# kkaytekin/Supervised-Depth-Estimation-from-Polarized-Images

Hardware: AMD Instinct MI355X
Metric: train images/sec (512x612, 3-encoder) (higher is better)
Workload: dtype f32; 1 GPU; BASELINE configs[2]: full 3-encoder (augment_xolp+augment_normals), multi-scale loss scales=[0,1,2,3], batch 16 per GPU, 512x612 frames (network/loss on 512x640 padded), dropout 0.1, Adam lr 1e-4, fp32; global_batch=16, height=512, width=640, frame_width=612, parallelism=dp1

## Files before the change

### supervised-depth-estimation-from-polarized-images_amd/csrc/elementwise.hip

```cpp
#include "pd_common.h"
#include <cstdlib>
#include <cstdint>

namespace {

constexpr int EW_T = 256;

__device__ __forceinline__ float4 ld4(const float* p) { return *reinterpret_cast<const float4*>(p); }
__device__ __forceinline__ void st4(float* p, float4 v) { *reinterpret_cast<float4*>(p) = v; }
typedef float ew_f4 __attribute__((ext_vector_type(4)));
__device__ __forceinline__ void st4_nt(float* p, float4 v) {
    const ew_f4 w = {v.x, v.y, v.z, v.w};
    __builtin_nontemporal_store(w, reinterpret_cast<ew_f4*>(p));
}
__device__ __forceinline__ float4 f4(float v) { return make_float4(v, v, v, v); }

__device__ __forceinline__ uint4 philox4x32_10(uint4 c, uint2 k) {
    const uint32_t M0 = 0xD2511F53u, M1 = 0xCD9E8D57u, W0 = 0x9E3779B9u, W1 = 0xBB67AE85u;
#pragma unroll
    for (int r = 0; r < 10; ++r) {
        const uint32_t hi0 = __umulhi(M0, c.x), lo0 = M0 * c.x;
        const uint32_t hi1 = __umulhi(M1, c.z), lo1 = M1 * c.z;
        c = make_uint4(hi1 ^ c.y ^ k.x, lo1, hi0 ^ c.w ^ k.y, lo0);
        k.x += W0; k.y += W1;
// ... 251 lines not shown
    if (a.pool) {
        const float* p = a.x + (((size_t)n * a.H + 2 * ho) * a.W + 2 * wo) * a.C + c4;
        float4 v[4];
        v[0] = affine4(ld4(p), s, b); v[1] = affine4(ld4(p + a.C), s, b);
        v[2] = affine4(ld4(p + (long)a.W * a.C), s, b); v[3] = affine4(ld4(p + (long)a.W * a.C + a.C), s, b);
        if (a.relu_pre) { v[0] = relu4(v[0]); v[1] = relu4(v[1]); v[2] = relu4(v[2]); v[3] = relu4(v[3]); }
        const int me = ((h & 1) << 1) | (w & 1);
        int ax = 0, ay = 0, az = 0, aw = 0;
        float mx = v[0].x, my = v[0].y, mz = v[0].z, mw = v[0].w;
#pragma unroll
        for (int j = 1; j < 4; ++j) {
            if (v[j].x > mx) { mx = v[j].x; ax = j; }
            if (v[j].y > my) { my = v[j].y; ay = j; }
            if (v[j].z > mz) { mz = v[j].z; az = j; }
            if (v[j].w > mw) { mw = v[j].w; aw = j; }
        }
        g = make_float4(ax == me ? g.x : 0.f, ay == me ? g.y : 0.f, az == me ? g.z : 0.f, aw == me ? g.w : 0.f);
    }
    if (a.relu_pre)
        g = make_float4(z.x > 0.f ? g.x : 0.f, z.y > 0.f ? g.y : 0.f, z.z > 0.f ? g.z : 0.f, z.w > 0.f ? g.w : 0.f);
    return g;
}

template <bool APPLY>
__global__ __launch_bounds__(EW_T) void chain_bwd_kernel(const ChainArgs a) {
    const unsigned cq = a.C >> 2;
    const unsigned total = (unsigned)a.N * a.H * a.W * cq;
    float4 sg = f4(0.f), sgx = f4(0.f);
    const unsigned i0 = blockIdx.x * (unsigned)EW_T + threadIdx.x;
    const int c4 = (int)(i0 % cq) * 4;
    const float4 s = a.scale ? ld4(a.scale + c4) : f4(1.f);
    const float4 b = a.scale ? ld4(a.shift + c4) : f4(0.f);
    const float4 m = a.mean ? ld4(a.mean + c4) : f4(0.f), is = a.mean ? ld4(a.invstd + c4) : f4(0.f);
    const float4 c1 = (APPLY && a.mean) ? ld4(a.coef + c4) : f4(0.f), c2 = (APPLY && a.mean) ? ld4(a.coef + a.C + c4) : f4(0.f);
    if (a.pool && !(a.H & 1) && !(a.W & 1)) {
        const unsigned Ho = a.H >> 1, Wo = a.W >> 1;
        const unsigned wtotal = (unsigned)a.N * Ho * Wo * cq;
        for (unsigned i = i0; i < wtotal; i += gridDim.x * (unsigned)EW_T) {
            const unsigned opix = i / cq;
            const unsigned t = opix / Wo;
            const unsigned wo = opix - t * Wo;
            const unsigned n = t / Ho;
            const unsigned ho = t - n * Ho;
            const size_t p00 = (((size_t)n * a.H + 2 * ho) * a.W + 2 * wo) * a.C + c4;
            const size_t offs[4] = {p00, p00 + a.C, p00 + (size_t)a.W * a.C, p00 + (size_t)a.W * a.C + a.C};
            float4 xv[4], v[4];
#pragma unroll
            for (int j = 0; j < 4; ++j) {
                xv[j] = ld4(a.x + offs[j]);
                v[j] = affine4(xv[j], s, b);
                if (a.relu_pre) v[j] = relu4(v[j]);
            }
            float4 g = ld4(a.dy + (size_t)opix * a.ld_dy + c4);
            if (a.relu_post) {
                const float4 o = ld4(a.out + (size_t)opix * a.ld_out + c4);
                g = make_float4(o.x > 0.f ? g.x : 0.f, o.y > 0.f ? g.y : 0.f, o.z > 0.f ? g.z : 0.f, o.w > 0.f ? g.w : 0.f);
            }
            if (a.drop_p > 0.f) g = mul4(g, dropout_scale(i, a.seed, site_offset(a.offset, a.step_state), a.drop_p));
            int ax = 0, ay = 0, az = 0, aw = 0;
            float mx = v[0].x, my = v[0].y, mz = v[0].z, mw = v[0].w;
#pragma unroll
            for (int j = 1; j < 4; ++j) {
                if (v[j].x > mx) { mx = v[j].x; ax = j; }
                if (v[j].y > my) { my = v[j].y; ay = j; }
                if (v[j].z > mz) { mz = v[j].z; az = j; }
                if (v[j].w > mw) { mw = v[j].w; aw = j; }
            }
            if (a.relu_pre)
                g = make_float4(mx > 0.f ? g.x : 0.f, my > 0.f ? g.y : 0.f, mz > 0.f ? g.z : 0.f, mw > 0.f ? g.w : 0.f);
#pragma unroll
            for (int j = 0; j < 4; ++j) {
                const float4 gj = make_float4(ax == j ? g.x : 0.f, ay == j ? g.y : 0.f, az == j ? g.z : 0.f, aw == j ? g.w : 0.f);
                float4 xh = f4(0.f);
                if (a.mean) xh = make_float4((xv[j].x - m.x) * is.x, (xv[j].y - m.y) * is.y, (xv[j].z - m.z) * is.z, (xv[j].w - m.w) * is.w);
                if (!APPLY) {
                    sg = add4(sg, gj);
                    sgx = add4(sgx, mul4(gj, xh));
                } else {
                    float4 d;
                    if (a.mean) d = make_float4(s.x * (gj.x - c1.x - xh.x * c2.x), s.y * (gj.y - c1.y - xh.y * c2.y),
                                                s.z * (gj.z - c1.z - xh.z * c2.z), s.w * (gj.w - c1.w - xh.w * c2.w));
                    else d = mul4(gj, s);
                    st4_nt(a.dx + offs[j], d);
                }
            }
        }
    } else
    for (unsigned i = i0; i < total; i += gridDim.x * (unsigned)EW_T) {
        const unsigned pix = i / cq;
        const unsigned t = pix / a.W;
        const unsigned w = pix - t * a.W;
        const unsigned n = t / a.H;
        const unsigned h = t - n * a.H;
        const float4 xv = ld4(a.x + (size_t)pix * a.C + c4);
        float4 gp;
        const float4 g = chain_grad(a, n, h, w, c4, xv, s, b, &gp);
        if (APPLY && a.dres) st4(a.dres + (size_t)pix * a.C + c4, gp);
        float4 xh = f4(0.f);
        if (a.mean) xh = make_float4((xv.x - m.x) * is.x, (xv.y - m.y) * is.y, (xv.z - m.z) * is.z, (xv.w - m.w) * is.w);
        if (!APPLY) {
            sg = add4(sg, g);
            sgx = add4(sgx, mul4(g, xh));
        } else {
            float4 d;
            if (a.mean) {
                d = make_float4(s.x * (g.x - c1.x - xh.x * c2.x), s.y * (g.y - c1.y - xh.y * c2.y),
                                s.z * (g.z - c1.z - xh.z * c2.z), s.w * (g.w - c1.w - xh.w * c2.w));
            } else {
                d = mul4(g, s);
            }
            st4_nt(a.dx + (size_t)pix * a.C + c4, d);
        }
    }
    if (!APPLY) {
        __shared__ float red[EW_T][8];
        float* r = red[threadIdx.x];
        r[0] = sg.x; r[1] = sg.y; r[2] = sg.z; r[3] = sg.w; r[4] = sgx.x; r[5] = sgx.y; r[6] = sgx.z; r[7] = sgx.w;
        __syncthreads();
        if ((int)threadIdx.x < cq) {
            float acc8[8] = {0, 0, 0, 0, 0, 0, 0, 0};
            for (int t = threadIdx.x; t < EW_T; t += cq)
#pragma unroll
                for (int j = 0; j < 8; ++j) acc8[j] += red[t][j];
            float* o = a.partial + ((long)blockIdx.x * a.C + 4 * threadIdx.x) * 2;
#pragma unroll
            for (int j = 0; j < 4; ++j) { o[2 * j] = acc8[j]; o[2 * j + 1] = acc8[4 + j]; }
        }
    }
}

__device__ __forceinline__ long divmod(long i, int d, int& rem) {
    if (i >> 32) { const long q = i / d; rem = (int)(i - q * d); return q; }
    const unsigned u = (unsigned)i, q = u / (unsigned)d;
    rem = (int)(u - q * (unsigned)d);
// ... 747 lines not shown
```

### supervised-depth-estimation-from-polarized-images_amd/csrc/loss.hip

```cpp
#include "pd_common.h"
#include <algorithm>
#include <cstdlib>

namespace {

constexpr int LT = 256;

__device__ __forceinline__ float wave_sum(float v) {
#pragma unroll
    for (int o = 32; o > 0; o >>= 1) v += __shfl_xor(v, o);
    return v;
}

template <int K>
__device__ __forceinline__ void block_sum(float (&v)[K], float* smem ) {
#pragma unroll
    for (int k = 0; k < K; ++k) v[k] = wave_sum(v[k]);
    const int lane = threadIdx.x & 63, wave = threadIdx.x >> 6;
    if (lane == 0)
#pragma unroll
        for (int k = 0; k < K; ++k) smem[wave * K + k] = v[k];
    __syncthreads();
    if (threadIdx.x == 0)
#pragma unroll
// ... 600 lines not shown
                                                      int N, long P, int accumulate, unsigned bid, unsigned nb) {
    const long total = N * P;
    for (long i = bid * (long)LT + threadIdx.x; i < total; i += (long)nb * LT) {
        const long n = i / P;
        if (!mean) { gdisp[i] = accumulate ? gdisp[i] + G[i] : G[i]; continue; }
        const float me = mean[n] + 1e-7f;
        const float v = G[i] / me - (float)(gd_acc[n] / ((double)me * me * (double)P));
        gdisp[i] = accumulate ? gdisp[i] + v : v;
    }
}
__global__ __launch_bounds__(LT) void smooth_bwd_final_kernel(const float* __restrict__ G, const float* __restrict__ mean,
                                                              const double* __restrict__ gd_acc, float* __restrict__ gdisp,
                                                              int N, long P, int accumulate) {
    smooth_bwd_final_body(G, mean, gd_acc, gdisp, N, P, accumulate, blockIdx.x, gridDim.x);
}

struct MsArgs {
    int S, N, H, W;
    const float* disp[8]; const float* color[8];
    float* depth[8]; float* mean[8]; float2* edge[8];
    float* gdisp[8]; float* gws[8]; float* gup[8];
    int hs[8], ws[8];
    unsigned nb_full, nb_s[8];
};

__global__ __launch_bounds__(LT) void ms_disp_to_depth_kernel(const MsArgs a, float min_disp, float max_disp) {
    const int s = blockIdx.y;
    disp_to_depth_body(a.disp[s], a.depth[s], nullptr, a.N, a.hs[s], a.ws[s], a.H, a.W, min_disp, max_disp, blockIdx.x, gridDim.x);
}

__global__ __launch_bounds__(LT) void ms_sup_fwd_kernel(const MsArgs a, const float* __restrict__ gt, const float* __restrict__ K,
                                                        const float4* __restrict__ gtn, float* __restrict__ partial,
                                                        int part_stride, float min_d, float max_d, int with_normals) {
    __shared__ float sm[4 * 3];
    const int N = a.N, H = a.H, W = a.W;
    const long total = (long)N * H * W;
    float acc[8][3];
#pragma unroll
    for (int s = 0; s < 8; ++s) { acc[s][0] = 0.f; acc[s][1] = 0.f; acc[s][2] = 0.f; }
    for (long i = blockIdx.x * (long)LT + threadIdx.x; i < total; i += (long)gridDim.x * LT) {
        int x, y;
        const long t = divmod(i, W, x);
        const long n = divmod(t, H, y);
        const float g = gt[i];
        if (!(g >= min_d && g <= max_d)) continue;
        V3 ng{0, 0, 0};
        float n1 = 1.f;
        Cam c{};
        if (with_normals) {
            c = load_cam(K, n);
            if (gtn) { const float4 q = gtn[i]; ng = V3{q.x, q.y, q.z}; }
            else { V3 A, B; float nv; sobel_xyz(gt + n * H * W, H, W, x, y, c, A, B); ng = normalize12(cross(A, B), nv); }
            n1 = fmaxf(sqrtf(dot(ng, ng)), 1e-8f);
        }
#pragma unroll
        for (int s = 0; s < 8; ++s) {
            if (s >= a.S) break;
            const float* pred = a.depth[s];
            acc[s][0] += fabsf(g - pred[i]);
            acc[s][2] += 1.f;
            if (with_normals) {
                V3 A, B; float nv;
                sobel_xyz(pred + n * H * W, H, W, x, y, c, A, B);
                const V3 np_ = normalize12(cross(A, B), nv);
                const float n2 = fmaxf(sqrtf(dot(np_, np_)), 1e-8f);
                const float cs = (ng.x / n1) * (np_.x / n2) + (ng.y / n1) * (np_.y / n2) + (ng.z / n1) * (np_.z / n2);
                acc[s][1] += 2.f - cs;
            }
        }
    }
    for (int s = 0; s < a.S; ++s) {
        float v[3] = {acc[s][0], acc[s][1], acc[s][2]};
        __syncthreads();
        block_sum<3>(v, sm);
        if (threadIdx.x == 0) {
            float* p = partial + ((long)s * part_stride + blockIdx.x) * 3;
            p[0] = v[0]; p[1] = v[1]; p[2] = v[2];
        }
    }
}

__global__ __launch_bounds__(1024) void ms_image_mean_kernel(const MsArgs a) {
    __shared__ double sm[16];
    const int s = blockIdx.y;
    image_mean_body(sm, a.disp[s], a.mean[s], a.hs[s] * a.ws[s], blockIdx.x);
}

__global__ __launch_bounds__(LT) void ms_smooth_fwd_kernel(const MsArgs a, float* __restrict__ partial, int part_stride) {
    __shared__ float sm[4 * 2];
    const int s = blockIdx.y;
    if (blockIdx.x >= a.nb_s[s]) return;
    smooth_fwd_body(sm, a.disp[s], a.color[s], a.mean[s], partial + (long)s * part_stride * 2, a.edge[s], a.N, a.hs[s], a.ws[s],
                    blockIdx.x, a.nb_s[s]);
}

__global__ __launch_bounds__(LT) void ms_sup_bwd_kernel(const MsArgs a, const float* __restrict__ gt, const float* __restrict__ K,
                                                        const float4* __restrict__ gtn, const float* __restrict__ wts,
                                                        const double* __restrict__ sums, float min_d, float max_d,
                                                        float disp_range, int tiles_h, int tiles_w, int ntiles) {
    __shared__ float abl[6][SB_HP];
    const int s = blockIdx.y;
    sup_bwd_fused_body(abl, a.depth[s], gt, K, gtn, wts + 3 * s, sums + 5 * s, a.gup[s], a.N, a.H, a.W, min_d, max_d, disp_range, 1,
                       tiles_h, tiles_w, ntiles, blockIdx.x, gridDim.x);
}

__global__ __launch_bounds__(LT) void ms_up_gather_bwd_kernel(const MsArgs a) {
    const int s = blockIdx.y;
    if (blockIdx.x >= a.nb_s[s]) return;
    const int f = a.H / a.hs[s];
    if (f == 1) up_gather_bwd_f_body<1>(a.gup[s], a.gdisp[s], a.N, a.hs[s], a.ws[s], a.H, a.W, 0, blockIdx.x, a.nb_s[s]);
    else if (f == 2) up_gather_bwd_f_body<2>(a.gup[s], a.gdisp[s], a.N, a.hs[s], a.ws[s], a.H, a.W, 0, blockIdx.x, a.nb_s[s]);
    else if (f == 4) up_gather_bwd_f_body<4>(a.gup[s], a.gdisp[s], a.N, a.hs[s], a.ws[s], a.H, a.W, 0, blockIdx.x, a.nb_s[s]);
    else up_gather_bwd_f_body<8>(a.gup[s], a.gdisp[s], a.N, a.hs[s], a.ws[s], a.H, a.W, 0, blockIdx.x, a.nb_s[s]);
}

__global__ __launch_bounds__(LT) void ms_smooth_bwd_g_kernel(const MsArgs a, const float* __restrict__ wts,
                                                             double* __restrict__ gd_acc) {
    __shared__ double smd[4];
    const int s = blockIdx.y;
    if (blockIdx.x >= a.nb_s[s]) return;
    smooth_bwd_g_body(smd, a.disp[s], a.color[s], a.mean[s], wts + 3 * s, a.edge[s], a.gws[s], gd_acc + (long)s * a.N, a.N,
                      a.hs[s], a.ws[s], blockIdx.x, a.nb_s[s]);
}

__global__ __launch_bounds__(LT) void ms_smooth_bwd_final_kernel(const MsArgs a, const double* __restrict__ gd_acc) {
    const int s = blockIdx.y;
    if (blockIdx.x >= a.nb_s[s]) return;
    smooth_bwd_final_body(a.gws[s], a.mean[s], gd_acc + (long)s * a.N, a.gdisp[s], a.N, (long)a.hs[s] * a.ws[s], 1, blockIdx.x,
                          a.nb_s[s]);
}

struct LossMeta {
    int S;
    int sup_rows[8], sm_rows[8], N[8], h[8], w[8], scale_id[8];
};

__global__ __launch_bounds__(256) void loss_finalize_kernel(const float* __restrict__ sup_part,
                                                            const float* __restrict__ sm_part, const LossMeta m,
                                                            int part_stride, float w_normals, float w_smooth,
                                                            double* __restrict__ sums, float* __restrict__ vals) {
    __shared__ double red[256];
    __shared__ double tot[8 * 5];
    for (int s = 0; s < m.S; ++s) {
        for (int j = 0; j < 5; ++j) {
            double v = 0.0;
            if (j < 3) {
                const float* sp = sup_part + (long)s * part_stride * 3;
                for (int r = threadIdx.x; r < m.sup_rows[s]; r += 256) v += sp[r * 3 + j];
            } else {
                const float* mp = sm_part + (long)s * part_stride * 2;
                for (int r = threadIdx.x; r < m.sm_rows[s]; r += 256) v += mp[r * 2 + (j - 3)];
            }
// ... 52 lines not shown
    wts[3 * s + 2] = gl * w_smooth / (float)(1 << m.scale_id[s]);
}

}

extern "C" int pd_loss_rows(long n) { return (int)lgrid(n); }

extern "C" int pd_disp_to_depth(const void* disp, void* depth, void* updisp, int N, int hs, int ws, int H, int W,
                                float min_depth, float max_depth, void* stream) {
    PD_REQUIRE(disp && depth && N >= 0 && hs > 0 && ws > 0 && H >= hs && W >= ws, "pd_disp_to_depth: bad arguments");
    PD_REQUIRE(min_depth > 0 && max_depth > min_depth, "pd_disp_to_depth: bad depth range");
    if (N == 0) return PD_OK;
    hipLaunchKernelGGL(disp_to_depth_kernel, dim3(lgrid((long)N * H * W)), dim3(LT), 0, (hipStream_t)stream,
                       (const float*)disp, (float*)depth, (float*)updisp, N, hs, ws, H, W, 1.f / max_depth,
                       1.f / min_depth);
    return pd::check_launch("pd_disp_to_depth");
}

extern "C" int pd_up_gather_bwd(const void* gup, void* gdisp, int N, int hs, int ws, int H, int W, int accumulate,
                                int generic, void* stream) {
    PD_REQUIRE(gup && gdisp && N >= 0 && hs > 0 && ws > 0, "pd_up_gather_bwd: bad arguments");
    PD_REQUIRE(H % hs == 0 && W % ws == 0, "pd_up_gather_bwd: full size must be an integer multiple of the scale size");
    if (N == 0) return PD_OK;
    const int f = generic ? 0 : H / hs;
    const unsigned grid = lgrid((long)N * hs * ws);
#define PD_UPG(F) hipLaunchKernelGGL(up_gather_bwd_f_kernel<F>, dim3(grid), dim3(LT), 0, (hipStream_t)stream, \
                                     (const float*)gup, (float*)gdisp, N, hs, ws, H, W, accumulate)
    if (W / ws == f && f == 1) PD_UPG(1);
    else if (W / ws == f && f == 2) PD_UPG(2);
    else if (W / ws == f && f == 4) PD_UPG(4);
    else if (W / ws == f && f == 8) PD_UPG(8);
    else
        hipLaunchKernelGGL(up_gather_bwd_kernel, dim3(grid), dim3(LT), 0, (hipStream_t)stream, (const float*)gup,
                           (float*)gdisp, N, hs, ws, H, W, accumulate);
#undef PD_UPG
    return pd::check_launch("pd_up_gather_bwd");
}

extern "C" int pd_gt_normals(const void* gt, const void* K, void* gtn, int N, int H, int W, float min_depth,
                             float max_depth, void* stream) {
    PD_REQUIRE(gt && K && gtn && N > 0 && H > 0 && W > 0 && pd::aligned16(gtn), "pd_gt_normals: bad arguments");
    hipLaunchKernelGGL(gt_normals_kernel, dim3(lgrid((long)N * H * W)), dim3(LT), 0, (hipStream_t)stream, (const float*)gt,
                       (const float*)K, (float4*)gtn, N, H, W, min_depth, max_depth);
    return pd::check_launch("pd_gt_normals");
}

extern "C" int pd_sup_loss_fwd(const void* pred, const void* gt, const void* K, const void* gt_normals, void* partial, int N,
                               int H, int W, float min_depth, float max_depth, int with_normals, void* stream) {
// ... 90 lines not shown
    const unsigned grid = lgrid((long)N * h * w);
    hipLaunchKernelGGL(smooth_bwd_g_kernel, dim3(grid), dim3(LT), 0, st, (const float*)disp, (const float*)img,
                       (const float*)mean, (const float*)wts, (const float2*)edge_w, (float*)g_ws, (double*)gd_acc, N, h, w);
    hipLaunchKernelGGL(smooth_bwd_final_kernel, dim3(grid), dim3(LT), 0, st, (const float*)g_ws, (const float*)mean,
                       (const double*)gd_acc, (float*)gdisp, N, (long)h * w, accumulate);
    return pd::check_launch("pd_smooth_bwd");
}

static int ms_fill(MsArgs& a, const void* const* disps, const void* const* colors, void* const* depths, void* const* means,
                   void* const* edge_ws, const int* hs, const int* ws, int S, int N, int H, int W) {
    PD_REQUIRE(S > 0 && S <= 8 && N > 0 && H > 0 && W > 0 && disps && depths && hs && ws, "pd_multiscale_loss: bad arguments");
    a = MsArgs{};
    a.S = S; a.N = N; a.H = H; a.W = W;
    a.nb_full = lgrid((long)N * H * W);
    for (int s = 0; s < S; ++s) {
        PD_REQUIRE(disps[s] && depths[s] && hs[s] > 1 && ws[s] > 1 && H % hs[s] == 0 && W % ws[s] == 0 && H / hs[s] == W / ws[s] &&
                       (H / hs[s] == 1 || H / hs[s] == 2 || H / hs[s] == 4 || H / hs[s] == 8),
                   "pd_multiscale_loss: scale %d: the full size must be 1, 2, 4 or 8 times the scale size", s);
        a.disp[s] = (const float*)disps[s]; a.color[s] = colors ? (const float*)colors[s] : nullptr;
        a.depth[s] = (float*)depths[s]; a.mean[s] = means ? (float*)means[s] : nullptr;
        a.edge[s] = edge_ws ? (float2*)edge_ws[s] : nullptr;
        a.hs[s] = hs[s]; a.ws[s] = ws[s];
        a.nb_s[s] = lgrid((long)N * hs[s] * ws[s]);
    }
    return PD_OK;
}

extern "C" int pd_multiscale_loss_fwd(const void* const* disps, const void* const* colors, const int* hs, const int* ws, int S,
                                      const void* gt, const void* K, const void* gt_normals, void* const* depths,
                                      void* const* means, void* const* edge_ws, void* sup_part, void* sm_part, int part_stride,
                                      int N, int H, int W, float min_depth, float max_depth, int with_normals, void* stream) {
    MsArgs a;
    int rc = ms_fill(a, disps, colors, depths, means, edge_ws, hs, ws, S, N, H, W);
    if (rc) return rc;
    PD_REQUIRE(colors && means && gt && (K || !with_normals) && sup_part && sm_part, "pd_multiscale_loss_fwd: null pointer");
    PD_REQUIRE(min_depth > 0 && max_depth > min_depth, "pd_multiscale_loss_fwd: bad depth range");
    unsigned nb_max = 0;
    for (int s = 0; s < S; ++s) { PD_REQUIRE(colors[s] && means[s], "pd_multiscale_loss_fwd: null scale tensor"); nb_max = std::max(nb_max, a.nb_s[s]); }
    PD_REQUIRE((int)a.nb_full <= part_stride && (int)nb_max <= part_stride, "pd_multiscale_loss_fwd: part_stride too small");
    hipStream_t st = (hipStream_t)stream;
    hipLaunchKernelGGL(ms_disp_to_depth_kernel, dim3(a.nb_full, S), dim3(LT), 0, st, a, 1.f / max_depth, 1.f / min_depth);
    hipLaunchKernelGGL(ms_sup_fwd_kernel, dim3(a.nb_full), dim3(LT), 0, st, a, (const float*)gt, (const float*)K,
                       (const float4*)gt_normals, (float*)sup_part, part_stride, min_depth, max_depth, with_normals);
    hipLaunchKernelGGL(ms_image_mean_kernel, dim3(N, S), dim3(1024), 0, st, a);
    hipLaunchKernelGGL(ms_smooth_fwd_kernel, dim3(nb_max, S), dim3(LT), 0, st, a, (float*)sm_part, part_stride);
    return pd::check_launch("pd_multiscale_loss_fwd");
}

extern "C" int pd_multiscale_loss_bwd(const void* const* disps, const void* const* colors, const void* const* depths,
                                      const void* const* means, const void* const* edge_ws, const int* hs, const int* ws, int S,
                                      const void* gt, const void* K, const void* gt_normals, const void* wts, const void* sums,
                                      void* gup_ws, void* g_ws, void* gd_acc, void* const* gdisps, int N, int H, int W,
                                      float min_depth, float max_depth, void* stream) {
    MsArgs a;
    int rc = ms_fill(a, disps, colors, const_cast<void* const*>(depths), const_cast<void* const*>(means),
                     const_cast<void* const*>(edge_ws), hs, ws, S, N, H, W);
    if (rc) return rc;
    PD_REQUIRE(colors && means && gt && K && wts && sums && gup_ws && g_ws && gd_acc && gdisps, "pd_multiscale_loss_bwd: null pointer");
    unsigned nb_max = 0;
    long goff = 0;
    for (int s = 0; s < S; ++s) {
        PD_REQUIRE(colors[s] && means[s] && gdisps[s], "pd_multiscale_loss_bwd: null scale tensor");
        a.gdisp[s] = (float*)gdisps[s];
        a.gup[s] = (float*)gup_ws + (long)s * N * H * W;
        a.gws[s] = (float*)g_ws + goff;
        goff += (long)N * hs[s] * ws[s];
        nb_max = std::max(nb_max, a.nb_s[s]);
    }
    hipStream_t st = (hipStream_t)stream;
    const int tiles_h = (H + SB_TR - 1) / SB_TR, tiles_w = (W + SB_TW - 1) / SB_TW;
    const long ntiles = (long)N * tiles_h * tiles_w;
    PD_REQUIRE(ntiles < (1L << 31), "pd_multiscale_loss_bwd: too many tiles");
    hipLaunchKernelGGL(ms_sup_bwd_kernel, dim3((unsigned)(ntiles > 4096 ? 4096 : ntiles), S), dim3(LT), 0, st, a, (const float*)gt,
                       (const float*)K, (const float4*)gt_normals, (const float*)wts, (const double*)sums, min_depth, max_depth,
                       1.f / min_depth - 1.f / max_depth, tiles_h, tiles_w, (int)ntiles);
    hipLaunchKernelGGL(ms_up_gather_bwd_kernel, dim3(nb_max, S), dim3(LT), 0, st, a);
    if (hipMemsetAsync(gd_acc, 0, sizeof(double) * N * S, st) != hipSuccess) return pd::fail(PD_ELAUNCH, "pd_multiscale_loss_bwd: memset");
    hipLaunchKernelGGL(ms_smooth_bwd_g_kernel, dim3(nb_max, S), dim3(LT), 0, st, a, (const float*)wts, (double*)gd_acc);
    hipLaunchKernelGGL(ms_smooth_bwd_final_kernel, dim3(nb_max, S), dim3(LT), 0, st, a, (const double*)gd_acc);
    return pd::check_launch("pd_multiscale_loss_bwd");
}

extern "C" int pd_loss_finalize(const void* sup_part, const int* sup_rows, const void* sm_part, const int* sm_rows,
                                const int* dims , const int* scale_ids, int S, int part_stride,
                                float w_normals, float w_smooth, void* sums, void* vals, void* stream) {
    PD_REQUIRE(sup_part && sup_rows && sm_part && sm_rows && dims && scale_ids && sums && vals && S > 0 && S <= 8,
               "pd_loss_finalize: bad arguments");
    LossMeta m{};
    m.S = S;
    for (int s = 0; s < S; ++s) {
        m.sup_rows[s] = sup_rows[s]; m.sm_rows[s] = sm_rows[s];
        m.N[s] = dims[3 * s]; m.h[s] = dims[3 * s + 1]; m.w[s] = dims[3 * s + 2]; m.scale_id[s] = scale_ids[s];
        PD_REQUIRE(sup_rows[s] <= part_stride && sm_rows[s] <= part_stride, "pd_loss_finalize: rows exceed part_stride");
    }
    hipLaunchKernelGGL(loss_finalize_kernel, dim3(1), dim3(256), 0, (hipStream_t)stream, (const float*)sup_part,
                       (const float*)sm_part, m, part_stride, w_normals, w_smooth, (double*)sums, (float*)vals);
    return pd::check_launch("pd_loss_finalize");
}

// ... 220 lines not shown
```

Baseline: 344.9 images/s.

## Tile multiscale loss kernels in shared memory and unroll chain-backward reduction loads

Replaces the multiscale supervised forward, supervised backward and upsample-gather backward loss kernels with shared-memory tiled versions. The forward pass stages depth rows per scale so Sobel taps are not re-read from global memory, and the backward pass handles all scales in one tiled launch. Separately, the chain-backward reduction pass batches several independent loads per thread before using them to raise memory-level parallelism. These changes add code complexity and shared-memory pressure, and the tiling assumes the integer upsample factors 1, 2, 4 and 8.

```diff
diff --git a/supervised-depth-estimation-from-polarized-images_amd/csrc/elementwise.hip b/supervised-depth-estimation-from-polarized-images_amd/csrc/elementwise.hip
--- a/supervised-depth-estimation-from-polarized-images_amd/csrc/elementwise.hip
+++ b/supervised-depth-estimation-from-polarized-images_amd/csrc/elementwise.hip
@@ -297,41 +297,60 @@
     return g;
 }
 
+#ifndef PD_CHAIN_RED_U
+#define PD_CHAIN_RED_U 2
+#endif
+#ifndef PD_CHAIN_RED_UW
+#define PD_CHAIN_RED_UW 1
+#endif
+constexpr int CHAIN_RED_U = PD_CHAIN_RED_U;
+constexpr int CHAIN_RED_UW = PD_CHAIN_RED_UW;
+struct ChainWin { unsigned i; size_t offs[4]; float4 xv[4], g, o; };
+struct ChainEl { unsigned i; float4 xv, g, o; };
+
 template <bool APPLY>
 __global__ __launch_bounds__(EW_T) void chain_bwd_kernel(const ChainArgs a) {
     const unsigned cq = a.C >> 2;
     const unsigned total = (unsigned)a.N * a.H * a.W * cq;
     float4 sg = f4(0.f), sgx = f4(0.f);
     const unsigned i0 = blockIdx.x * (unsigned)EW_T + threadIdx.x;
+    const unsigned stride = gridDim.x * (unsigned)EW_T;
     const int c4 = (int)(i0 % cq) * 4;
     const float4 s = a.scale ? ld4(a.scale + c4) : f4(1.f);
     const float4 b = a.scale ? ld4(a.shift + c4) : f4(0.f);
     const float4 m = a.mean ? ld4(a.mean + c4) : f4(0.f), is = a.mean ? ld4(a.invstd + c4) : f4(0.f);
     const float4 c1 = (APPLY && a.mean) ? ld4(a.coef + c4) : f4(0.f), c2 = (APPLY && a.mean) ? ld4(a.coef + a.C + c4) : f4(0.f);
+    constexpr int U = APPLY ? 1 : CHAIN_RED_U, UW = APPLY ? 1 : CHAIN_RED_UW;
     if (a.pool && !(a.H & 1) && !(a.W & 1)) {
         const unsigned Ho = a.H >> 1, Wo = a.W >> 1;
         const unsigned wtotal = (unsigned)a.N * Ho * Wo * cq;
-        for (unsigned i = i0; i < wtotal; i += gridDim.x * (unsigned)EW_T) {
+        auto load = [&](unsigned i, ChainWin& q) {
+            q.i = i;
             const unsigned opix = i / cq;
             const unsigned t = opix / Wo;
             const unsigned wo = opix - t * Wo;
             const unsigned n = t / Ho;
             const unsigned ho = t - n * Ho;
             const size_t p00 = (((size_t)n * a.H + 2 * ho) * a.W + 2 * wo) * a.C + c4;
-            const size_t offs[4] = {p00, p00 + a.C, p00 + (size_t)a.W * a.C, p00 + (size_t)a.W * a.C + a.C};
-            float4 xv[4], v[4];
+            q.offs[0] = p00; q.offs[1] = p00 + a.C; q.offs[2] = p00 + (size_t)a.W * a.C; q.offs[3] = p00 + (size_t)a.W * a.C + a.C;
+#pragma unroll
+            for (int j = 0; j < 4; ++j) q.xv[j] = ld4(a.x + q.offs[j]);
+            q.g = ld4(a.dy + (size_t)opix * a.ld_dy + c4);
+            q.o = a.relu_post ? ld4(a.out + (size_t)opix * a.ld_out + c4) : f4(0.f);
+        };
+        auto use = [&](const ChainWin& q) {
+            float4 v[4];
 #pragma unroll
             for (int j = 0; j < 4; ++j) {
-                xv[j] = ld4(a.x + offs[j]);
-                v[j] = affine4(xv[j], s, b);
+                v[j] = affine4(q.xv[j], s, b);
                 if (a.relu_pre) v[j] = relu4(v[j]);
             }
-            float4 g = ld4(a.dy + (size_t)opix * a.ld_dy + c4);
+            float4 g = q.g;
             if (a.relu_post) {
-                const float4 o = ld4(a.out + (size_t)opix * a.ld_out + c4);
+                const float4 o = q.o;
                 g = make_float4(o.x > 0.f ? g.x : 0.f, o.y > 0.f ? g.y : 0.f, o.z > 0.f ? g.z : 0.f, o.w > 0.f ? g.w : 0.f);
             }
-            if (a.drop_p > 0.f) g = mul4(g, dropout_scale(i, a.seed, site_offset(a.offset, a.step_state), a.drop_p));
+            if (a.drop_p > 0.f) g = mul4(g, dropout_scale(q.i, a.seed, site_offset(a.offset, a.step_state), a.drop_p));
             int ax = 0, ay = 0, az = 0, aw = 0;
             float mx = v[0].x, my = v[0].y, mz = v[0].z, mw = v[0].w;
 #pragma unroll
@@ -347,7 +366,7 @@
             for (int j = 0; j < 4; ++j) {
                 const float4 gj = make_float4(ax == j ? g.x : 0.f, ay == j ? g.y : 0.f, az == j ? g.z : 0.f, aw == j ? g.w : 0.f);
                 float4 xh = f4(0.f);
-                if (a.mean) xh = make_float4((xv[j].x - m.x) * is.x, (xv[j].y - m.y) * is.y, (xv[j].z - m.z) * is.z, (xv[j].w - m.w) * is.w);
+                if (a.mean) xh = make_float4((q.xv[j].x - m.x) * is.x, (q.xv[j].y - m.y) * is.y, (q.xv[j].z - m.z) * is.z, (q.xv[j].w - m.w) * is.w);
                 if (!APPLY) {
                     sg = add4(sg, gj);
                     sgx = add4(sgx, mul4(gj, xh));
@@ -356,35 +375,83 @@
                     if (a.mean) d = make_float4(s.x * (gj.x - c1.x - xh.x * c2.x), s.y * (gj.y - c1.y - xh.y * c2.y),
                                                 s.z * (gj.z - c1.z - xh.z * c2.z), s.w * (gj.w - c1.w - xh.w * c2.w));
                     else d = mul4(gj, s);
-                    st4_nt(a.dx + offs[j], d);
+                    st4_nt(a.dx + q.offs[j], d);
                 }
             }
-        }
-    } else
-    for (unsigned i = i0; i < total; i += gridDim.x * (unsigned)EW_T) {
-        const unsigned pix = i / cq;
-        const unsigned t = pix / a.W;
-        const unsigned w = pix - t * a.W;
-        const unsigned n = t / a.H;
-        const unsigned h = t - n * a.H;
-        const float4 xv = ld4(a.x + (size_t)pix * a.C + c4);
-        float4 gp;
-        const float4 g = chain_grad(a, n, h, w, c4, xv, s, b, &gp);
-        if (APPLY && a.dres) st4(a.dres + (size_t)pix * a.C + c4, gp);
-        float4 xh = f4(0.f);
-        if (a.mean) xh = make_float4((xv.x - m.x) * is.x, (xv.y - m.y) * is.y, (xv.z - m.z) * is.z, (xv.w - m.w) * is.w);
-        if (!APPLY) {
-            sg = add4(sg, g);
-            sgx = add4(sgx, mul4(g, xh));
-        } else {
-            float4 d;
-            if (a.mean) {
-                d = make_float4(s.x * (g.x - c1.x - xh.x * c2.x), s.y * (g.y - c1.y - xh.y * c2.y),
-                                s.z * (g.z - c1.z - xh.z * c2.z), s.w * (g.w - c1.w - xh.w * c2.w));
+        };
+        unsigned i = i0;
+        if (UW > 1) {
+            for (; i + (UW - 1) * stride < wtotal; i += UW * stride) {
+                ChainWin q[UW];
+#pragma unroll
+                for (int u = 0; u < UW; ++u) load(i + u * stride, q[u]);
+#pragma unroll
+                for (int u = 0; u < UW; ++u) use(q[u]);
+            }
+        }
+        for (; i < wtotal; i += stride) {
+            ChainWin q;
+            load(i, q);
+            use(q);
+        }
+    } else {
+        unsigned i = i0;
+        if (U > 1 && !a.pool) {
+            auto load = [&](unsigned e, ChainEl& q) {
+                q.i = e;
+                const unsigned pix = e / cq;
+                q.xv = ld4(a.x + (size_t)pix * a.C + c4);
+                q.g = ld4(a.dy + (size_t)pix * a.ld_dy + c4);
+                q.o = a.relu_post ? ld4(a.out + (size_t)pix * a.ld_out + c4) : f4(0.f);
+            };
+            auto use = [&](const ChainEl& q) {
+                float4 g = q.g;
+                if (a.relu_post) {
+                    const float4 o = q.o;
+                    g = make_float4(o.x > 0.f ? g.x : 0.f, o.y > 0.f ? g.y : 0.f, o.z > 0.f ? g.z : 0.f, o.w > 0.f ? g.w : 0.f);
+                }
+                if (a.drop_p > 0.f) g = mul4(g, dropout_scale(q.i, a.seed, site_offset(a.offset, a.step_state), a.drop_p));
+                const float4 z = affine4(q.xv, s, b);
+                if (a.relu_pre)
+                    g = make_float4(z.x > 0.f ? g.x : 0.f, z.y > 0.f ? g.y : 0.f, z.z > 0.f ? g.z : 0.f, z.w > 0.f ? g.w : 0.f);
+                float4 xh = f4(0.f);
+                if (a.mean) xh = make_float4((q.xv.x - m.x) * is.x, (q.xv.y - m.y) * is.y, (q.xv.z - m.z) * is.z, (q.xv.w - m.w) * is.w);
+                sg = add4(sg, g);
+                sgx = add4(sgx, mul4(g, xh));
+            };
+            for (; i + (U - 1) * stride < total; i += U * stride) {
+                ChainEl q[U];
+#pragma unroll
+                for (int u = 0; u < U; ++u) load(i + u * stride, q[u]);
+#pragma unroll
+                for (int u = 0; u < U; ++u) use(q[u]);
+            }
+        }
+        for (; i < total; i += stride) {
+            const unsigned pix = i / cq;
+            const unsigned t = pix / a.W;
+            const unsigned w = pix - t * a.W;
+            const unsigned n = t / a.H;
+            const unsigned h = t - n * a.H;
+            const float4 xv = ld4(a.x + (size_t)pix * a.C + c4);
+            float4 gp;
+            const float4 g = chain_grad(a, n, h, w, c4, xv, s, b, &gp);
+            if (APPLY && a.dres) st4(a.dres + (size_t)pix * a.C + c4, gp);
+            float4 xh = f4(0.f);
+            if (a.mean) xh = make_float4((xv.x - m.x) * is.x, (xv.y - m.y) * is.y, (xv.z - m.z) * is.z, (xv.w - m.w) * is.w);
+            if (!APPLY) {
+                sg = add4(sg, g);
+                sgx = add4(sgx, mul4(g, xh));
             } else {
-                d = mul4(g, s);
-            }
-            st4_nt(a.dx + (size_t)pix * a.C + c4, d);
+                float4 d;
+                if (a.mean) {
+                    d = make_float4(s.x * (g.x - c1.x - xh.x * c2.x), s.y * (g.y - c1.y - xh.y * c2.y),
+                                    s.z * (g.z - c1.z - xh.z * c2.z), s.w * (g.w - c1.w - xh.w * c2.w));
+                } else {
+                    d = mul4(g, s);
+                }
+                st4_nt(a.dx + (size_t)pix * a.C + c4, d);
+            }
         }
     }
     if (!APPLY) {
diff --git a/supervised-depth-estimation-from-polarized-images_amd/csrc/loss.hip b/supervised-depth-estimation-from-polarized-images_amd/csrc/loss.hip
--- a/supervised-depth-estimation-from-polarized-images_amd/csrc/loss.hip
+++ b/supervised-depth-estimation-from-polarized-images_amd/csrc/loss.hip
@@ -646,62 +646,12 @@
     float* gdisp[8]; float* gws[8]; float* gup[8];
     int hs[8], ws[8];
     unsigned nb_full, nb_s[8];
+    unsigned nb_tiles[8];
 };
 
 __global__ __launch_bounds__(LT) void ms_disp_to_depth_kernel(const MsArgs a, float min_disp, float max_disp) {
     const int s = blockIdx.y;
     disp_to_depth_body(a.disp[s], a.depth[s], nullptr, a.N, a.hs[s], a.ws[s], a.H, a.W, min_disp, max_disp, blockIdx.x, gridDim.x);
-}
-
-__global__ __launch_bounds__(LT) void ms_sup_fwd_kernel(const MsArgs a, const float* __restrict__ gt, const float* __restrict__ K,
-                                                        const float4* __restrict__ gtn, float* __restrict__ partial,
-                                                        int part_stride, float min_d, float max_d, int with_normals) {
-    __shared__ float sm[4 * 3];
-    const int N = a.N, H = a.H, W = a.W;
-    const long total = (long)N * H * W;
-    float acc[8][3];
-#pragma unroll
-    for (int s = 0; s < 8; ++s) { acc[s][0] = 0.f; acc[s][1] = 0.f; acc[s][2] = 0.f; }
-    for (long i = blockIdx.x * (long)LT + threadIdx.x; i < total; i += (long)gridDim.x * LT) {
-        int x, y;
-        const long t = divmod(i, W, x);
-        const long n = divmod(t, H, y);
-        const float g = gt[i];
-        if (!(g >= min_d && g <= max_d)) continue;
-        V3 ng{0, 0, 0};
-        float n1 = 1.f;
-        Cam c{};
-        if (with_normals) {
-            c = load_cam(K, n);
-            if (gtn) { const float4 q = gtn[i]; ng = V3{q.x, q.y, q.z}; }
-            else { V3 A, B; float nv; sobel_xyz(gt + n * H * W, H, W, x, y, c, A, B); ng = normalize12(cross(A, B), nv); }
-            n1 = fmaxf(sqrtf(dot(ng, ng)), 1e-8f);
-        }
-#pragma unroll
-        for (int s = 0; s < 8; ++s) {
-            if (s >= a.S) break;
-            const float* pred = a.depth[s];
-            acc[s][0] += fabsf(g - pred[i]);
-            acc[s][2] += 1.f;
-            if (with_normals) {
-                V3 A, B; float nv;
-                sobel_xyz(pred + n * H * W, H, W, x, y, c, A, B);
-                const V3 np_ = normalize12(cross(A, B), nv);
-                const float n2 = fmaxf(sqrtf(dot(np_, np_)), 1e-8f);
-                const float cs = (ng.x / n1) * (np_.x / n2) + (ng.y / n1) * (np_.y / n2) + (ng.z / n1) * (np_.z / n2);
-                acc[s][1] += 2.f - cs;
-            }
-        }
-    }
-    for (int s = 0; s < a.S; ++s) {
-        float v[3] = {acc[s][0], acc[s][1], acc[s][2]};
-        __syncthreads();
-        block_sum<3>(v, sm);
-        if (threadIdx.x == 0) {
-            float* p = partial + ((long)s * part_stride + blockIdx.x) * 3;
-            p[0] = v[0]; p[1] = v[1]; p[2] = v[2];
-        }
-    }
 }
 
 __global__ __launch_bounds__(1024) void ms_image_mean_kernel(const MsArgs a) {
@@ -716,26 +666,6 @@
     if (blockIdx.x >= a.nb_s[s]) return;
     smooth_fwd_body(sm, a.disp[s], a.color[s], a.mean[s], partial + (long)s * part_stride * 2, a.edge[s], a.N, a.hs[s], a.ws[s],
                     blockIdx.x, a.nb_s[s]);
-}
-
-__global__ __launch_bounds__(LT) void ms_sup_bwd_kernel(const MsArgs a, const float* __restrict__ gt, const float* __restrict__ K,
-                                                        const float4* __restrict__ gtn, const float* __restrict__ wts,
-                                                        const double* __restrict__ sums, float min_d, float max_d,
-                                                        float disp_range, int tiles_h, int tiles_w, int ntiles) {
-    __shared__ float abl[6][SB_HP];
-    const int s = blockIdx.y;
-    sup_bwd_fused_body(abl, a.depth[s], gt, K, gtn, wts + 3 * s, sums + 5 * s, a.gup[s], a.N, a.H, a.W, min_d, max_d, disp_range, 1,
-                       tiles_h, tiles_w, ntiles, blockIdx.x, gridDim.x);
-}
-
-__global__ __launch_bounds__(LT) void ms_up_gather_bwd_kernel(const MsArgs a) {
-    const int s = blockIdx.y;
-    if (blockIdx.x >= a.nb_s[s]) return;
-    const int f = a.H / a.hs[s];
-    if (f == 1) up_gather_bwd_f_body<1>(a.gup[s], a.gdisp[s], a.N, a.hs[s], a.ws[s], a.H, a.W, 0, blockIdx.x, a.nb_s[s]);
-    else if (f == 2) up_gather_bwd_f_body<2>(a.gup[s], a.gdisp[s], a.N, a.hs[s], a.ws[s], a.H, a.W, 0, blockIdx.x, a.nb_s[s]);
-    else if (f == 4) up_gather_bwd_f_body<4>(a.gup[s], a.gdisp[s], a.N, a.hs[s], a.ws[s], a.H, a.W, 0, blockIdx.x, a.nb_s[s]);
-    else up_gather_bwd_f_body<8>(a.gup[s], a.gdisp[s], a.N, a.hs[s], a.ws[s], a.H, a.W, 0, blockIdx.x, a.nb_s[s]);
 }
 
 __global__ __launch_bounds__(LT) void ms_smooth_bwd_g_kernel(const MsArgs a, const float* __restrict__ wts,
@@ -752,6 +682,319 @@
     if (blockIdx.x >= a.nb_s[s]) return;
     smooth_bwd_final_body(a.gws[s], a.mean[s], gd_acc + (long)s * a.N, a.gdisp[s], a.N, (long)a.hs[s] * a.ws[s], 1, blockIdx.x,
                           a.nb_s[s]);
+}
+
+
+template <class DTap>
+__device__ __forceinline__ void sobel_xyz_taps(DTap&& dtap, const float (&u)[3], const float (&v)[3], V3& A, V3& B) {
+    A = V3{0, 0, 0}; B = V3{0, 0, 0};
+#pragma unroll
+    for (int dy = -1; dy <= 1; ++dy) {
+        const float sy = dy == 0 ? 2.f : 1.f, ddy = (float)dy;
+#pragma unroll
+        for (int dx = -1; dx <= 1; ++dx) {
+            const float sx = dx == 0 ? 2.f : 1.f, ddx = (float)dx;
+            const float d = dtap(dy, dx);
+            const float X = u[dx + 1] * d, Y = v[dy + 1] * d;
+            const float kx = sy * ddx * 0.125f, ky = ddy * sx * 0.125f;
+            A.x += kx * X; A.y += kx * Y; A.z += kx * d;
+            B.x += ky * X; B.y += ky * Y; B.z += ky * d;
+        }
+    }
+}
+
+__device__ __forceinline__ void normals_grad_from_ab(V3 A, V3 B, V3 gh, float wln, V3& dA, V3& dB) {
+    float nv;
+    const V3 v = cross(A, B);
+    const V3 nn = normalize12(v, nv);
+    const float nl = sqrtf(dot(nn, nn));
+    V3 wn;
+    if (nl > 1e-8f) {
+        const float inv = 1.f / nl, pr = dot(gh, nn) * inv * inv * inv;
+        wn = V3{-wln * (gh.x * inv - pr * nn.x), -wln * (gh.y * inv - pr * nn.y), -wln * (gh.z * inv - pr * nn.z)};
+    } else {
+        wn = V3{-wln * gh.x * 1e8f, -wln * gh.y * 1e8f, -wln * gh.z * 1e8f};
+    }
+    V3 wv;
+    if (nv > 1e-12f) {
+        const float inv = 1.f / nv, pr = dot(wn, nn);
+        wv = V3{(wn.x - pr * nn.x) * inv, (wn.y - pr * nn.y) * inv, (wn.z - pr * nn.z) * inv};
+    } else {
+        wv = V3{wn.x * 1e12f, wn.y * 1e12f, wn.z * 1e12f};
+    }
+    dA = cross(B, wv);
+    dB = cross(wv, A);
+}
+
+constexpr int SF_SEG = LT + 2;
+__global__ __launch_bounds__(LT) void ms_sup_fwd_tiled_kernel(const MsArgs a, const float* __restrict__ gt,
+                                                              const float* __restrict__ K, const float4* __restrict__ gtn,
+                                                              float* __restrict__ partial, int part_stride, float min_d,
+                                                              float max_d, int with_normals) {
+    __shared__ float sm[4 * 3];
+    __shared__ float seg[8][3][SF_SEG];
+    const int N = a.N, H = a.H, W = a.W, S = a.S;
+    const long total = (long)N * H * W;
+    float acc[8][3];
+#pragma unroll
+    for (int s = 0; s < 8; ++s) { acc[s][0] = 0.f; acc[s][1] = 0.f; acc[s][2] = 0.f; }
+    for (long f0 = blockIdx.x * (long)LT; f0 < total; f0 += (long)gridDim.x * LT) {
+        __syncthreads();
+        for (int e = threadIdx.x; e < S * 3 * SF_SEG; e += LT) {
+            const int s = e / (3 * SF_SEG), r = e - s * (3 * SF_SEG);
+            const int j = r / SF_SEG, p = r - j * SF_SEG;
+            const long t = f0 + (long)(j - 1) * W + p - 1;
+            seg[s][j][p] = (t >= 0 && t < total) ? a.depth[s][t] : 0.f;
+        }
+        __syncthreads();
+        const long i = f0 + threadIdx.x;
+        if (i >= total) continue;
+        const float g = gt[i];
+        if (!(g >= min_d && g <= max_d)) continue;
+        V3 gh{0, 0, 0};
+        float u[3] = {0.f, 0.f, 0.f}, v[3] = {0.f, 0.f, 0.f};
+        int ox[3] = {0, 0, 0}, oy[3] = {0, 0, 0};
+        if (with_normals) {
+            int x, y;
+            const long t = divmod(i, W, x);
+            const long n = divmod(t, H, y);
+            const Cam c = load_cam(K, n);
+            V3 ng;
+            if (gtn) { const float4 q = gtn[i]; ng = V3{q.x, q.y, q.z}; }
+            else { V3 A, B; float nv; sobel_xyz(gt + n * H * W, H, W, x, y, c, A, B); ng = normalize12(cross(A, B), nv); }
+            const float n1 = fmaxf(sqrtf(dot(ng, ng)), 1e-8f);
+            gh = V3{ng.x / n1, ng.y / n1, ng.z / n1};
+#pragma unroll
+            for (int d = -1; d <= 1; ++d) {
+                const int xx = min(max(x + d, 0), W - 1), yy = min(max(y + d, 0), H - 1);
+                u[d + 1] = (xx - c.cx) / c.fx; v[d + 1] = (yy - c.cy) / c.fy;
+                ox[d + 1] = xx - x; oy[d + 1] = yy - y;
+            }
+        }
+#pragma unroll
+        for (int s = 0; s < 8; ++s) {
+            if (s >= S) break;
+            acc[s][0] += fabsf(g - seg[s][1][threadIdx.x + 1]);
+            acc[s][2] += 1.f;
+            if (with_normals) {
+                V3 A, B; float nv;
+                sobel_xyz_taps([&](int dy, int dx) { return seg[s][1 + oy[dy + 1]][threadIdx.x + 1 + ox[dx + 1]]; }, u, v, A, B);
+                const V3 np_ = normalize12(cross(A, B), nv);
+                const float n2 = fmaxf(sqrtf(dot(np_, np_)), 1e-8f);
+                const float cs = gh.x * (np_.x / n2) + gh.y * (np_.y / n2) + gh.z * (np_.z / n2);
+                acc[s][1] += 2.f - cs;
+            }
+        }
+    }
+    for (int s = 0; s < S; ++s) {
+        float v[3] = {acc[s][0], acc[s][1], acc[s][2]};
+        __syncthreads();
+        block_sum<3>(v, sm);
+        if (threadIdx.x == 0) {
+            float* p = partial + ((long)s * part_stride + blockIdx.x) * 3;
+            p[0] = v[0]; p[1] = v[1]; p[2] = v[2];
+        }
+    }
+}
+
+constexpr int ST_R = SB_TR + 4, ST_C = SB_TW + 4;
+struct SupTile {
+    float dl[ST_R * ST_C];
+    float abl[6][SB_HP];
+    float ghl[3][SB_HP];
+    float gl[SB_HP];
+    float ul[ST_C], vl[ST_R];
+    float twx[SB_TW][3][2], twy[SB_TR][3][2];
+};
+__global__ __launch_bounds__(LT) void ms_sup_bwd_tiled_kernel(const MsArgs a, const float* __restrict__ gt,
+                                                              const float* __restrict__ K, const float4* __restrict__ gtn,
+                                                              const float* __restrict__ wts, const double* __restrict__ sums,
+                                                              float min_d, float max_d, float disp_range, int tiles_h,
+                                                              int tiles_w, int ntiles) {
+    __shared__ SupTile L;
+    const int H = a.H, W = a.W;
+    for (int tile = (int)blockIdx.x; tile < ntiles; tile += (int)gridDim.x) {
+        const int tw = tile % tiles_w, th = (tile / tiles_w) % tiles_h;
+        const long n = tile / (tiles_w * tiles_h);
+        const int h0 = th * SB_TR, w0 = tw * SB_TW;
+        const Cam c = load_cam(K, n);
+        const float* gn = gt + n * H * W;
+        __syncthreads();
+        for (int s = threadIdx.x; s < SB_HP; s += LT) {
+            const int r = s / SB_HC, cc = s - r * SB_HC;
+            const int y = h0 - 1 + r, x = w0 - 1 + cc;
+            float g = __builtin_nanf("");
+            V3 gh{0, 0, 0};
+            if (y >= 0 && y < H && x >= 0 && x < W) {
+                const long i = (n * H + y) * (long)W + x;
+                g = gt[i];
+                if (g >= min_d && g <= max_d) {
+                    V3 ng;
+                    if (gtn) { const float4 q = gtn[i]; ng = V3{q.x, q.y, q.z}; }
+                    else { V3 Ag, Bg; float nvg; sobel_xyz(gn, H, W, x, y, c, Ag, Bg); ng = normalize12(cross(Ag, Bg), nvg); }
+                    const float n1 = fmaxf(sqrtf(dot(ng, ng)), 1e-8f);
+                    gh = V3{ng.x / n1, ng.y / n1, ng.z / n1};
+                }
+            }
+            L.gl[s] = g; L.ghl[0][s] = gh.x; L.ghl[1][s] = gh.y; L.ghl[2][s] = gh.z;
+        }
+        for (int j = threadIdx.x; j < ST_C; j += LT) { const int xx = min(max(w0 - 2 + j, 0), W - 1); L.ul[j] = (xx - c.cx) / c.fx; }
+        for (int j = threadIdx.x; j < ST_R; j += LT) { const int yy = min(max(h0 - 2 + j, 0), H - 1); L.vl[j] = (yy - c.cy) / c.fy; }
+        for (int j = threadIdx.x; j < SB_TW * 3; j += LT) {
+            const int cc = j / 3, t = j - cc * 3, x = w0 + cc, px = x - 1 + t;
+            float wd = 0.f, ws = 0.f;
+            if (x < W && px >= 0 && px < W) tap_weights(x, px, W, wd, ws);
+            L.twx[cc][t][0] = wd; L.twx[cc][t][1] = ws;
+        }
+        for (int j = threadIdx.x; j < SB_TR * 3; j += LT) {
+            const int r = j / 3, t = j - r * 3, y = h0 + r, py = y - 1 + t;
+            float wd = 0.f, ws = 0.f;
+            if (y < H && py >= 0 && py < H) tap_weights(y, py, H, wd, ws);
+            L.twy[r][t][0] = wd; L.twy[r][t][1] = ws;
+        }
+        for (int sc = 0; sc < a.S; ++sc) {
+            const float* pn = a.depth[sc] + n * H * W;
+            float* gout = a.gup[sc];
+            const float wln = (float)((double)wts[3 * sc + 1] / sums[5 * sc + 2]);
+            const float wl1 = (float)((double)wts[3 * sc] / sums[5 * sc + 2]);
+            __syncthreads();
+            for (int e = threadIdx.x; e < ST_R * ST_C; e += LT) {
+                const int r = e / ST_C, cc = e - r * ST_C;
+                const int yy = min(max(h0 - 2 + r, 0), H - 1), xx = min(max(w0 - 2 + cc, 0), W - 1);
+                L.dl[e] = pn[(long)yy * W + xx];
+            }
+            __syncthreads();
+            for (int s = threadIdx.x; s < SB_HP; s += LT) {
+                const int r = s / SB_HC, cc = s - r * SB_HC;
+                const float g = L.gl[s];
+                V3 dA{0, 0, 0}, dB{0, 0, 0};
+                if (g >= min_d && g <= max_d) {
+                    const float u[3] = {L.ul[cc], L.ul[cc + 1], L.ul[cc + 2]}, v[3] = {L.vl[r], L.vl[r + 1], L.vl[r + 2]};
+                    const float* dc = L.dl + (r + 1) * ST_C + cc + 1;
+                    V3 A, B;
+                    sobel_xyz_taps([&](int dy, int dx) { return dc[dy * ST_C + dx]; }, u, v, A, B);
+                    normals_grad_from_ab(A, B, V3{L.ghl[0][s], L.ghl[1][s], L.ghl[2][s]}, wln, dA, dB);
+                }
+                L.abl[0][s] = dA.x; L.abl[1][s] = dA.y; L.abl[2][s] = dA.z; L.abl[3][s] = dB.x; L.abl[4][s] = dB.y; L.abl[5][s] = dB.z;
+            }
+            __syncthreads();
+            for (int o = threadIdx.x; o < SB_TR * SB_TW; o += LT) {
+                const int r = o / SB_TW, cc = o - r * SB_TW;
+                const int y = h0 + r, x = w0 + cc;
+                if (y >= H || x >= W) continue;
+                const long i = (n * H + y) * (long)W + x;
+                const float g = L.gl[(r + 1) * SB_HC + cc + 1], d = L.dl[(r + 2) * ST_C + cc + 2];
+                float gd = 0.f;
+                if (g >= min_d && g <= max_d) gd = wl1 * (d > g ? 1.f : (d < g ? -1.f : 0.f));
+                V3 s{0, 0, 0};
+#pragma unroll
+                for (int ty = 0; ty < 3; ++ty) {
+                    const int py = y - 1 + ty;
+                    if (py < 0 || py > H - 1) continue;
+                    const float dyw = L.twy[r][ty][0], syw = L.twy[r][ty][1];
+#pragma unroll
+                    for (int tx = 0; tx < 3; ++tx) {
+                        const int px = x - 1 + tx;
+                        if (px < 0 || px > W - 1) continue;
+                        const float dxw = L.twx[cc][tx][0], sxw = L.twx[cc][tx][1];
+                        const float ka = syw * dxw * 0.125f, kb = dyw * sxw * 0.125f;
+                        const int q = (r + ty) * SB_HC + cc + tx;
+                        s.x += ka * L.abl[0][q] + kb * L.abl[3][q]; s.y += ka * L.abl[1][q] + kb * L.abl[4][q];
+                        s.z += ka * L.abl[2][q] + kb * L.abl[5][q];
+                    }
+                }
+                gd += L.ul[cc + 2] * s.x + L.vl[r + 2] * s.y + s.z;
+                gout[i] = gd * (-disp_range * d * d);
+            }
+        }
+    }
+}
+
+constexpr int UG_R = 8, UG_C = 32;
+template <int F>
+__device__ __forceinline__ void up_gather_bwd_tiled_body(float* __restrict__ stage ,
+                                                         float* __restrict__ wyl ,
+                                                         const float* __restrict__ gup, float* __restrict__ gdisp, int N,
+                                                         int hs, int ws, int H, int W, int accumulate, unsigned tile) {
+    constexpr int Q = UG_C + 2;
+    const int tiles_w = (ws + UG_C - 1) / UG_C, tiles_h = (hs + UG_R - 1) / UG_R;
+    const int tw = tile % tiles_w, th = (tile / tiles_w) % tiles_h;
+    const long n = tile / (tiles_w * tiles_h);
+    const int ys0 = th * UG_R, xs0 = tw * UG_C;
+    const int xl = threadIdx.x % UG_C, yl = threadIdx.x / UG_C;
+    const int xs = xs0 + xl, ys = ys0 + yl;
+    const float sh = (float)hs / H, sw = (float)ws / W;
+    float wx[3 * F];
+#pragma unroll
+    for (int b = 0; b < 3 * F; ++b) {
+        const int x = (xs - 1) * F + b;
+        int x0, x1; float lx1;
+        src_index(x, sw, ws, x0, x1, lx1);
+        const float w = (x0 == xs ? 1.f - lx1 : 0.f) + (x1 == xs ? lx1 : 0.f);
+        wx[b] = (x >= 0 && x < W) ? w : 0.f;
+    }
+    for (int j = threadIdx.x; j < UG_R * 3 * F; j += LT) {
+        const int r = j / (3 * F), k = j - r * (3 * F);
+        const int yr = ys0 + r, y = (yr - 1) * F + k;
+        float w = 0.f;
+        if (y >= 0 && y < H) {
+            int y0, y1; float ly1;
+            src_index(y, sh, hs, y0, y1, ly1);
+            w = (y0 == yr ? 1.f - ly1 : 0.f) + (y1 == yr ? ly1 : 0.f);
+        }
+        wyl[j] = w;
+    }
+    float acc = 0.f;
+    for (int band = 0; band < UG_R + 2; ++band) {
+        const int yb = (ys0 - 1 + band) * F;
+        if (yb + F <= 0 || yb >= H) continue;
+        __syncthreads();
+        for (int e = threadIdx.x; e < F * F * Q; e += LT) {
+            const int ar = e / (F * Q), ci = e - ar * (F * Q);
+            const int y = yb + ar, x = (xs0 - 1) * F + ci;
+            const float v = (y >= 0 && y < H && x >= 0 && x < W) ? gup[(n * H + y) * (long)W + x] : 0.f;
+            stage[(ar * F + ci % F) * Q + ci / F] = v;
+        }
+        __syncthreads();
+        const int rel = band - yl;
+        if (rel < 0 || rel > 2) continue;
+#pragma unroll
+        for (int ar = 0; ar < F; ++ar) {
+            const int y = yb + ar;
+            if (y < 0 || y >= H) continue;
+            const float wy = wyl[yl * 3 * F + rel * F + ar];
+            if (wy == 0.f) continue;
+            const float* g = stage + ar * F * Q + xl;
+#pragma unroll
+            for (int b = 0; b < 3 * F; ++b)
+                if (wx[b] != 0.f) acc += wy * wx[b] * g[(b % F) * Q + b / F];
+        }
+    }
+    if (xs < ws && ys < hs) {
+        const long i = (n * hs + ys) * (long)ws + xs;
+        gdisp[i] = accumulate ? gdisp[i] + acc : acc;
+    }
+}
+inline long up_gather_tiles(int N, int hs, int ws) { return (long)N * ((hs + UG_R - 1) / UG_R) * ((ws + UG_C - 1) / UG_C); }
+
+template <int F>
+__global__ __launch_bounds__(LT) void up_gather_bwd_tiled_kernel(const float* __restrict__ gup, float* __restrict__ gdisp,
+                                                                 int N, int hs, int ws, int H, int W, int accumulate) {
+    __shared__ float stage[F * F * (UG_C + 2)];
+    __shared__ float wyl[UG_R * 3 * F];
+    up_gather_bwd_tiled_body<F>(stage, wyl, gup, gdisp, N, hs, ws, H, W, accumulate, blockIdx.x);
+}
+
+__global__ __launch_bounds__(LT) void ms_up_gather_bwd_tiled_kernel(const MsArgs a) {
+    __shared__ float stage[8 * 8 * (UG_C + 2)];
+    __shared__ float wyl[UG_R * 3 * 8];
+    const int s = blockIdx.y;
+    if (blockIdx.x >= a.nb_tiles[s]) return;
+    const int f = a.H / a.hs[s];
+    if (f == 1) up_gather_bwd_tiled_body<1>(stage, wyl, a.gup[s], a.gdisp[s], a.N, a.hs[s], a.ws[s], a.H, a.W, 0, blockIdx.x);
+    else if (f == 2) up_gather_bwd_tiled_body<2>(stage, wyl, a.gup[s], a.gdisp[s], a.N, a.hs[s], a.ws[s], a.H, a.W, 0, blockIdx.x);
+    else if (f == 4) up_gather_bwd_tiled_body<4>(stage, wyl, a.gup[s], a.gdisp[s], a.N, a.hs[s], a.ws[s], a.H, a.W, 0, blockIdx.x);
+    else up_gather_bwd_tiled_body<8>(stage, wyl, a.gup[s], a.gdisp[s], a.N, a.hs[s], a.ws[s], a.H, a.W, 0, blockIdx.x);
 }
 
 struct LossMeta {
@@ -850,8 +1093,20 @@
     PD_REQUIRE(gup && gdisp && N >= 0 && hs > 0 && ws > 0, "pd_up_gather_bwd: bad arguments");
     PD_REQUIRE(H % hs == 0 && W % ws == 0, "pd_up_gather_bwd: full size must be an integer multiple of the scale size");
     if (N == 0) return PD_OK;
-    const int f = generic ? 0 : H / hs;
+    const int f = generic == 1 ? 0 : H / hs;
     const unsigned grid = lgrid((long)N * hs * ws);
+    if (generic == 0 && W / ws == f && (f == 1 || f == 2 || f == 4 || f == 8)) {
+        const long tiles = up_gather_tiles(N, hs, ws);
+        PD_REQUIRE(tiles < (1L << 31), "pd_up_gather_bwd: too many tiles");
+#define PD_UPT(F) hipLaunchKernelGGL(up_gather_bwd_tiled_kernel<F>, dim3((unsigned)tiles), dim3(LT), 0, (hipStream_t)stream, \
+                                     (const float*)gup, (float*)gdisp, N, hs, ws, H, W, accumulate)
+        if (f == 1) PD_UPT(1);
+        else if (f == 2) PD_UPT(2);
+        else if (f == 4) PD_UPT(4);
+        else PD_UPT(8);
+#undef PD_UPT
+        return pd::check_launch("pd_up_gather_bwd");
+    }
 #define PD_UPG(F) hipLaunchKernelGGL(up_gather_bwd_f_kernel<F>, dim3(grid), dim3(LT), 0, (hipStream_t)stream, \
                                      (const float*)gup, (float*)gdisp, N, hs, ws, H, W, accumulate)
     if (W / ws == f && f == 1) PD_UPG(1);
@@ -988,6 +1243,8 @@
         a.edge[s] = edge_ws ? (float2*)edge_ws[s] : nullptr;
         a.hs[s] = hs[s]; a.ws[s] = ws[s];
         a.nb_s[s] = lgrid((long)N * hs[s] * ws[s]);
+        PD_REQUIRE(up_gather_tiles(N, hs[s], ws[s]) < (1L << 31), "pd_multiscale_loss: scale %d: too many tiles", s);
+        a.nb_tiles[s] = (unsigned)up_gather_tiles(N, hs[s], ws[s]);
     }
     return PD_OK;
 }
@@ -1006,7 +1263,7 @@
     PD_REQUIRE((int)a.nb_full <= part_stride && (int)nb_max <= part_stride, "pd_multiscale_loss_fwd: part_stride too small");
     hipStream_t st = (hipStream_t)stream;
     hipLaunchKernelGGL(ms_disp_to_depth_kernel, dim3(a.nb_full, S), dim3(LT), 0, st, a, 1.f / max_depth, 1.f / min_depth);
-    hipLaunchKernelGGL(ms_sup_fwd_kernel, dim3(a.nb_full), dim3(LT), 0, st, a, (const float*)gt, (const float*)K,
+    hipLaunchKernelGGL(ms_sup_fwd_tiled_kernel, dim3(a.nb_full), dim3(LT), 0, st, a, (const float*)gt, (const float*)K,
                        (const float4*)gt_normals, (float*)sup_part, part_stride, min_depth, max_depth, with_normals);
     hipLaunchKernelGGL(ms_image_mean_kernel, dim3(N, S), dim3(1024), 0, st, a);
     hipLaunchKernelGGL(ms_smooth_fwd_kernel, dim3(nb_max, S), dim3(LT), 0, st, a, (float*)sm_part, part_stride);
@@ -1023,7 +1280,7 @@
                      const_cast<void* const*>(edge_ws), hs, ws, S, N, H, W);
     if (rc) return rc;
     PD_REQUIRE(colors && means && gt && K && wts && sums && gup_ws && g_ws && gd_acc && gdisps, "pd_multiscale_loss_bwd: null pointer");
-    unsigned nb_max = 0;
+    unsigned nb_max = 0, nt_max = 0;
     long goff = 0;
     for (int s = 0; s < S; ++s) {
         PD_REQUIRE(colors[s] && means[s] && gdisps[s], "pd_multiscale_loss_bwd: null scale tensor");
@@ -1032,15 +1289,16 @@
         a.gws[s] = (float*)g_ws + goff;
         goff += (long)N * hs[s] * ws[s];
         nb_max = std::max(nb_max, a.nb_s[s]);
+        nt_max = std::max(nt_max, a.nb_tiles[s]);
     }
     hipStream_t st = (hipStream_t)stream;
     const int tiles_h = (H + SB_TR - 1) / SB_TR, tiles_w = (W + SB_TW - 1) / SB_TW;
     const long ntiles = (long)N * tiles_h * tiles_w;
     PD_REQUIRE(ntiles < (1L << 31), "pd_multiscale_loss_bwd: too many tiles");
-    hipLaunchKernelGGL(ms_sup_bwd_kernel, dim3((unsigned)(ntiles > 4096 ? 4096 : ntiles), S), dim3(LT), 0, st, a, (const float*)gt,
+    hipLaunchKernelGGL(ms_sup_bwd_tiled_kernel, dim3((unsigned)ntiles), dim3(LT), 0, st, a, (const float*)gt,
                        (const float*)K, (const float4*)gt_normals, (const float*)wts, (const double*)sums, min_depth, max_depth,
                        1.f / min_depth - 1.f / max_depth, tiles_h, tiles_w, (int)ntiles);
-    hipLaunchKernelGGL(ms_up_gather_bwd_kernel, dim3(nb_max, S), dim3(LT), 0, st, a);
+    hipLaunchKernelGGL(ms_up_gather_bwd_tiled_kernel, dim3(nt_max, S), dim3(LT), 0, st, a);
     if (hipMemsetAsync(gd_acc, 0, sizeof(double) * N * S, st) != hipSuccess) return pd::fail(PD_ELAUNCH, "pd_multiscale_loss_bwd: memset");
     hipLaunchKernelGGL(ms_smooth_bwd_g_kernel, dim3(nb_max, S), dim3(LT), 0, st, a, (const float*)wts, (double*)gd_acc);
     hipLaunchKernelGGL(ms_smooth_bwd_final_kernel, dim3(nb_max, S), dim3(LT), 0, st, a, (const double*)gd_acc);
```

Measured after the change: 345.7 images/s, median of 6. No clear change (+0.2%).
